# fwereade/trivy

Measured on AMD Instinct MI355X. Metric: packages matched/sec (node), higher is better.
Workload: dtype u8; 1 GPU; c2-dpkg-10000x400; packages=4000000, packages_rank0=4000000, matches_rank0=20482442, kernel_variant=fused_k4_m2400_wseg_rec_r16, db_keys=150005, db_advisories=1709707

## Files before the change

### include/trivy_amd.h

```cpp
#ifndef TRIVY_AMD_H
#define TRIVY_AMD_H

#include <stddef.h>
#include <stdint.h>

#ifdef __cplusplus
extern "C" {
#endif

#define TVM_ABI_VERSION 1

enum {
  TVM_OK = 0,
  TVM_EDETECT = 1,
  TVM_EUNSUPPORTED_OS = 2,
  TVM_EINVAL = 3,
  TVM_EDEVICE = 4,
  TVM_EUNSUPPORTED_TYPE = 5,
};

typedef struct tvm_db tvm_db;
typedef struct tvm_engine tvm_engine;
typedef struct tvm_batch tvm_batch;

// ... 95 lines not shown
int tvm_ospkg_is_supported(const char* os_family, const char* os_ver, int64_t now_unix);
void tvm_result_free(tvm_result* r);

const char* tvm_library_type(const char* lib_type);
int tvm_library_detect(tvm_engine* e, const char* lib_type, const tvm_package* pkgs, size_t n, tvm_result* out,
                       char* err, size_t errlen);
int tvm_library_detect_vulnerabilities(tvm_engine* e, const char* lib_type, tvm_str pkg_id, tvm_str pkg_name,
                                       tvm_str pkg_ver, tvm_result* out, char* err, size_t errlen);

tvm_batch* tvm_batch_new(void);
void tvm_batch_free(tvm_batch* b);
int64_t tvm_batch_add(tvm_batch* b, tvm_engine* e, const char* bucket, tvm_str name, tvm_str version);
enum { TVM_ATTR_ARCH = 1, TVM_ATTR_KSPLICE = 2, TVM_ATTR_CPESET = 4 };
int64_t tvm_batch_add_many_ex(tvm_batch* b, tvm_engine* e, const char* bucket, size_t n, const char* arena,
                              const uint64_t* name_off, const uint32_t* name_len, const uint64_t* ver_off,
                              const uint32_t* ver_len, const uint64_t* arch_off, const uint32_t* arch_len,
                              uint32_t flags);
int64_t tvm_batch_cpe_set(tvm_batch* b, tvm_engine* e, const tvm_str* content_sets, size_t n, tvm_str nvr);
typedef struct {
  const uint64_t* arch_off;
  const uint32_t* arch_len;
  const uint32_t* cpe_set;
} tvm_attr_cols;
int64_t tvm_batch_add_many_attrs(tvm_batch* b, tvm_engine* e, const char* bucket, size_t n, const char* arena,
                                 const uint64_t* name_off, const uint32_t* name_len, const uint64_t* ver_off,
                                 const uint32_t* ver_len, const tvm_attr_cols* attrs, uint32_t flags);
int64_t tvm_batch_add_many(tvm_batch* b, tvm_engine* e, const char* bucket, size_t n, const char* arena,
                           const uint64_t* name_off, const uint32_t* name_len, const uint64_t* ver_off,
                           const uint32_t* ver_len);
int64_t tvm_batch_add_targets(tvm_batch* b, tvm_engine* e, size_t n_targets, const tvm_str* buckets,
                              const uint64_t* target_end, const char* arena, const uint64_t* name_off,
                              const uint32_t* name_len, const uint64_t* ver_off, const uint32_t* ver_len);
int64_t tvm_batch_add_targets_attrs(tvm_batch* b, tvm_engine* e, size_t n_targets, const tvm_str* buckets,
                                    const uint32_t* target_flags, const uint64_t* target_end, const char* arena,
                                    const uint64_t* name_off, const uint32_t* name_len, const uint64_t* ver_off,
                                    const uint32_t* ver_len, const tvm_attr_cols* attrs);
int64_t tvm_batch_size(const tvm_batch* b);
int tvm_batch_upload(tvm_engine* e, tvm_batch* b, uint64_t match_cap, char* err, size_t errlen);
int tvm_match_launch(tvm_engine* e, tvm_batch* b, char* err, size_t errlen);
int tvm_engine_sync(tvm_engine* e, char* err, size_t errlen);
int tvm_device_sync(int device, char* err, size_t errlen);
void tvm_shutdown(void);
int tvm_match_status(tvm_engine* e, tvm_batch* b, uint64_t* n_matches, int64_t* err_pkg, uint64_t* err_bits);
int tvm_match_fetch(tvm_engine* e, tvm_batch* b, uint32_t* pairs, uint64_t cap, uint64_t* n_out);
int tvm_match_copy_device(tvm_engine* e, tvm_batch* b, void* dst, uint64_t cap, uint64_t* n_out);
int tvm_match_order_into(tvm_engine* e, tvm_batch* b, void* csr_adv_dev, void* row_end_dev, uint64_t cap,
                         uint64_t* n_out, char* err, size_t errlen);
int tvm_match_time(tvm_engine* e, tvm_batch* b, int steps, double* ms, char* err, size_t errlen);
uint64_t tvm_match_algorithmic_bytes(tvm_engine* e, tvm_batch* b);
int tvm_version_key(int grammar, const char* s, size_t n, uint8_t* out, size_t cap);
int tvm_version_class(int grammar, const char* s, size_t n);
int tvm_deb_fast_key_host(const char* s, size_t n, uint32_t shift, uint8_t* out, size_t cap);
int tvm_deb_fast_key_slot_host(const char* s, size_t n, uint32_t shift, uint8_t* kb, size_t kb_len);
enum { TVM_ISVULN_PAIRWISE = 0x100 };
int tvm_lib_is_vulnerable_host(int grammar, const char* ver, size_t ver_len, const char* advisory_json,
                               size_t json_len);
const char* tvm_db_advisory_vuln_id(const tvm_db* db, uint32_t adv);

int tvm_db_rows_many(const tvm_db* db, const char* bucket, size_t n, const char* arena, const uint64_t* name_off,
                     const uint32_t* name_len, uint32_t* out);
int tvm_batch_set_package_base(tvm_batch* b, uint32_t base);
int tvm_batch_upload_into(tvm_engine* e, tvm_batch* b, void* pkg_dev, void* adv_dev, uint64_t cap, char* err,
                          size_t errlen);

enum { TVM_PIPE_RAW = 1, TVM_PIPE_ADV32 = 2, TVM_PIPE_RH_MERGE = 4 };
int tvm_pipeline_prepare(tvm_engine* e, tvm_batch* b, uint64_t match_cap, uint32_t chunk_packages, uint32_t flags,
                         char* err, size_t errlen);
int tvm_pipeline_run(tvm_engine* e, tvm_batch* b, uint64_t* n_matches, int64_t* err_pkg, double* ms, char* err,
                     size_t errlen);
int tvm_pipeline_result(tvm_batch* b, const uint32_t** adv, const uint32_t** row_end, uint64_t* n_matches);
int tvm_pipeline_result_raw(tvm_batch* b, const void** adv, uint32_t* width, const uint32_t** row_end,
                            uint64_t* n_matches);
int tvm_pipeline_stats(tvm_batch* b, uint64_t out[5]);
int tvm_wire_encode(size_t n, const uint32_t* plat, const char* arena, const uint64_t* name_off, const uint32_t* name_len,
                    const uint64_t* ver_off, const uint32_t* ver_len, uint32_t chunk_packages, int threads, void* out,
                    uint64_t cap, uint64_t* bytes,
                    uint64_t* chunks, uint64_t chunks_cap, uint64_t* n_chunks, uint32_t* plats, uint32_t plats_cap,
                    uint32_t* n_plats);
int tvm_pipeline_times(tvm_batch* b, uint64_t* encode_us, uint64_t* prepare_us);
void tvm_pool_stats(uint64_t out[4]);
void tvm_pool_trim(void);
int tvm_runtime_info(int* hip_runtime, int* hip_driver, char* path, size_t pathlen);

typedef struct tvm_sbom tvm_sbom;
enum { TVM_SBOM_BORROW = 1 };
int tvm_sbom_decode_cyclonedx(const char* text, size_t len, uint32_t flags, tvm_sbom** out, char* err, size_t errlen);
void tvm_sbom_free(tvm_sbom* s);
int tvm_sbom_info(const tvm_sbom* s, int32_t* has_os, tvm_str* os_family, tvm_str* os_name, tvm_str* serial,
                  int64_t* version, size_t* n_apps);
int tvm_sbom_packages(const tvm_sbom* s, int64_t app, tvm_str* type, tvm_str* file_path, const tvm_package** pkgs,
                      size_t* n);
typedef struct {
  tvm_str purl, bom_ref, layer_digest, layer_diff_id;
  uint32_t present;
} tvm_sbom_extra;
int tvm_sbom_package_extra(const tvm_sbom* s, int64_t app, size_t i, tvm_sbom_extra* out);

int tvm_match_redhat_result(tvm_engine* e, tvm_batch* b, tvm_result* out, char* err, size_t errlen);
int tvm_match_redhat_merge(tvm_engine* e, tvm_batch* b, char* err, size_t errlen);
int tvm_match_redhat_vulns(tvm_engine* e, tvm_batch* b, const uint32_t* pairs, uint64_t n, tvm_result* out,
                           char* err, size_t errlen);
int tvm_match_redhat_merge_time(tvm_engine* e, tvm_batch* b, int steps, double* ms, char* err, size_t errlen);

typedef struct {
  const uint32_t* row_end;
  size_t n_pkgs;
// ... 94 lines not shown
```

### trivy_amd/_lib.py

```python
import atexit
import ctypes
import os

_HERE = os.path.dirname(os.path.abspath(__file__))
LIB_PATH = os.environ.get("TVM_LIB_PATH") or os.path.join(_HERE, "libtrivy_amd.so")

TVM_OK, TVM_EDETECT, TVM_EUNSUPPORTED_OS, TVM_EINVAL, TVM_EDEVICE, TVM_EUNSUPPORTED_TYPE = 0, 1, 2, 3, 4, 5
COPY_PKG_ID, COPY_PKG_NAME, COPY_IDENTIFIER, COPY_LAYER = 1, 2, 4, 8


class Str(ctypes.Structure):
    _fields_ = [("p", ctypes.c_char_p), ("n", ctypes.c_size_t)]


class Package(ctypes.Structure):
    _fields_ = [
        ("id", Str), ("name", Str), ("version", Str), ("release", Str), ("arch", Str),
        ("epoch", ctypes.c_int64),
        ("src_name", Str), ("src_version", Str), ("src_release", Str),
        ("src_epoch", ctypes.c_int64),
        ("modularitylabel", Str),
        ("has_build_info", ctypes.c_int32),
        ("content_sets", ctypes.POINTER(Str)), ("n_content_sets", ctypes.c_size_t),
        ("nvr", Str), ("build_arch", Str),
# ... 152 lines not shown
    ("tvm_engine_sync", ctypes.c_int, [_P, ctypes.c_char_p, ctypes.c_size_t]),
    ("tvm_device_sync", ctypes.c_int, [ctypes.c_int, ctypes.c_char_p, ctypes.c_size_t]),
    ("tvm_shutdown", None, []),
    ("tvm_pipeline_times", ctypes.c_int, [_P, ctypes.POINTER(ctypes.c_uint64), ctypes.POINTER(ctypes.c_uint64)]),
    ("tvm_pool_stats", None, [ctypes.POINTER(ctypes.c_uint64)]),
    ("tvm_sbom_decode_cyclonedx", ctypes.c_int, [ctypes.c_void_p, ctypes.c_size_t, ctypes.c_uint32,
                                                 ctypes.POINTER(ctypes.c_void_p),
                                                 ctypes.c_char_p, ctypes.c_size_t]),
    ("tvm_sbom_free", None, [ctypes.c_void_p]),
    ("tvm_sbom_info", ctypes.c_int, [ctypes.c_void_p, ctypes.POINTER(ctypes.c_int32), ctypes.POINTER(RawStr),
                                     ctypes.POINTER(RawStr), ctypes.POINTER(RawStr), ctypes.POINTER(ctypes.c_int64),
                                     ctypes.POINTER(ctypes.c_size_t)]),
    ("tvm_sbom_packages", ctypes.c_int, [ctypes.c_void_p, ctypes.c_int64, ctypes.POINTER(RawStr), ctypes.POINTER(RawStr),
                                         ctypes.POINTER(ctypes.POINTER(RawPackage)), ctypes.POINTER(ctypes.c_size_t)]),
    ("tvm_sbom_package_extra", ctypes.c_int, [ctypes.c_void_p, ctypes.c_int64, ctypes.c_size_t,
                                              ctypes.POINTER(SbomExtra)]),
    ("tvm_wire_encode", ctypes.c_int, [ctypes.c_size_t, ctypes.c_void_p, ctypes.c_char_p, ctypes.c_void_p,
                                       ctypes.c_void_p, ctypes.c_void_p, ctypes.c_void_p,
                                       ctypes.c_uint32, ctypes.c_int, ctypes.c_void_p, ctypes.c_uint64,
                                       ctypes.POINTER(ctypes.c_uint64), ctypes.c_void_p, ctypes.c_uint64,
                                       ctypes.POINTER(ctypes.c_uint64), ctypes.c_void_p, ctypes.c_uint32,
                                       ctypes.POINTER(ctypes.c_uint32)]),
    ("tvm_pool_trim", None, []),
    ("tvm_match_status", ctypes.c_int, [_P, _P, ctypes.POINTER(ctypes.c_uint64), ctypes.POINTER(ctypes.c_int64),
                                        ctypes.POINTER(ctypes.c_uint64)]),
    ("tvm_match_fetch", ctypes.c_int, [_P, _P, ctypes.c_void_p, ctypes.c_uint64, ctypes.POINTER(ctypes.c_uint64)]),
    ("tvm_match_copy_device", ctypes.c_int, [_P, _P, ctypes.c_void_p, ctypes.c_uint64, ctypes.POINTER(ctypes.c_uint64)]),
    ("tvm_match_order_into", ctypes.c_int, [_P, _P, ctypes.c_void_p, ctypes.c_void_p, ctypes.c_uint64,
                                            ctypes.POINTER(ctypes.c_uint64), ctypes.c_char_p, ctypes.c_size_t]),
    ("tvm_match_time", ctypes.c_int, [_P, _P, ctypes.c_int, ctypes.POINTER(ctypes.c_double), ctypes.c_char_p,
                                      ctypes.c_size_t]),
    ("tvm_match_algorithmic_bytes", ctypes.c_uint64, [_P, _P]),
    ("tvm_db_rows_many", ctypes.c_int, [_P, ctypes.c_char_p, ctypes.c_size_t, ctypes.c_void_p, ctypes.c_void_p,
                                        ctypes.c_void_p, ctypes.c_void_p]),
    ("tvm_batch_set_package_base", ctypes.c_int, [_P, ctypes.c_uint32]),
    ("tvm_batch_upload_into", ctypes.c_int, [_P, _P, ctypes.c_void_p, ctypes.c_void_p, ctypes.c_uint64,
                                             ctypes.c_char_p, ctypes.c_size_t]),
    ("tvm_pipeline_prepare", ctypes.c_int, [_P, _P, ctypes.c_uint64, ctypes.c_uint32, ctypes.c_uint32, ctypes.c_char_p,
                                            ctypes.c_size_t]),
    ("tvm_pipeline_run", ctypes.c_int, [_P, _P, ctypes.POINTER(ctypes.c_uint64), ctypes.POINTER(ctypes.c_int64),
                                        ctypes.POINTER(ctypes.c_double), ctypes.c_char_p, ctypes.c_size_t]),
    ("tvm_pipeline_result", ctypes.c_int, [_P, ctypes.POINTER(ctypes.c_void_p), ctypes.POINTER(ctypes.c_void_p),
                                           ctypes.POINTER(ctypes.c_uint64)]),
    ("tvm_pipeline_result_raw", ctypes.c_int, [_P, ctypes.POINTER(ctypes.c_void_p), ctypes.POINTER(ctypes.c_uint32),
                                               ctypes.POINTER(ctypes.c_void_p), ctypes.POINTER(ctypes.c_uint64)]),
    ("tvm_pipeline_stats", ctypes.c_int, [_P, ctypes.POINTER(ctypes.c_uint64)]),
    ("tvm_version_key", ctypes.c_int, [ctypes.c_int, ctypes.c_char_p, ctypes.c_size_t, ctypes.c_void_p,
                                       ctypes.c_size_t]),
    ("tvm_engine_dropin_stats", ctypes.c_int, [_P, ctypes.POINTER(ctypes.c_uint64)]),
    ("tvm_deb_fast_key_host", ctypes.c_int, [ctypes.c_char_p, ctypes.c_size_t, ctypes.c_uint32, ctypes.c_void_p,
                                             ctypes.c_size_t]),
    ("tvm_deb_fast_key_slot_host", ctypes.c_int, [ctypes.c_char_p, ctypes.c_size_t, ctypes.c_uint32, ctypes.c_void_p,
                                                  ctypes.c_size_t]),
    ("tvm_db_advisory_vuln_id", ctypes.c_char_p, [_P, ctypes.c_uint32]),
    ("tvm_version_class", ctypes.c_int, [ctypes.c_int, ctypes.c_char_p, ctypes.c_size_t]),
    ("tvm_lib_is_vulnerable_host", ctypes.c_int, [ctypes.c_int, ctypes.c_char_p, ctypes.c_size_t, ctypes.c_char_p,
                                                  ctypes.c_size_t]),
    ("tvm_library_type", ctypes.c_char_p, [ctypes.c_char_p]),
    ("tvm_library_detect", ctypes.c_int, [_P, ctypes.c_char_p, ctypes.POINTER(Package), ctypes.c_size_t,
                                          ctypes.POINTER(Result), ctypes.c_char_p, ctypes.c_size_t]),
    ("tvm_library_detect_vulnerabilities", ctypes.c_int, [_P, ctypes.c_char_p, Str, Str, Str, ctypes.POINTER(Result),
                                                          ctypes.c_char_p, ctypes.c_size_t]),
    ("tvm_fill_info", ctypes.c_int, [_P, ctypes.POINTER(FillIn), ctypes.c_size_t, ctypes.POINTER(FillResult),
                                     ctypes.c_char_p, ctypes.c_size_t]),
    ("tvm_fill_result_free", None, [ctypes.POINTER(FillResult)]),
    ("tvm_match_fill", ctypes.c_int, [_P, _P, ctypes.c_char_p, ctypes.c_size_t]),
    ("tvm_match_fill_fetch", ctypes.c_int, [_P, _P, ctypes.c_void_p, ctypes.c_uint64, ctypes.POINTER(ctypes.c_uint64)]),
    ("tvm_match_fill_time", ctypes.c_int, [_P, _P, ctypes.c_int, ctypes.POINTER(ctypes.c_double), ctypes.c_char_p,
                                           ctypes.c_size_t]),
    ("tvm_match_fill_algorithmic_bytes", ctypes.c_uint64, [_P, _P]),
    ("tvm_fill_source_name", ctypes.c_char_p, [_P, ctypes.c_uint32]),
    ("tvm_match_filter", ctypes.c_int, [_P, _P, ctypes.POINTER(FilterOpts), ctypes.POINTER(ctypes.c_uint64),
                                        ctypes.POINTER(ctypes.c_uint64), ctypes.c_char_p, ctypes.c_size_t]),
    ("tvm_match_filter_fetch", ctypes.c_int, [_P, _P, ctypes.c_void_p, ctypes.c_uint64,
                                              ctypes.POINTER(ctypes.c_uint64)]),
    ("tvm_match_filter_ignored", ctypes.c_int, [_P, _P, ctypes.c_void_p, ctypes.c_uint64,
                                                ctypes.POINTER(ctypes.c_uint64)]),
    ("tvm_vuln_rank_many", ctypes.c_int, [_P, ctypes.POINTER(Str), ctypes.c_size_t, ctypes.c_void_p]),
    ("tvm_batch_set_report", ctypes.c_int, [_P, ctypes.c_uint64, ctypes.c_uint64, ctypes.POINTER(Str),
                                            ctypes.POINTER(Str), ctypes.POINTER(Str)]),
    ("tvm_match_vulns", ctypes.c_int, [_P, _P, ctypes.POINTER(VulnSet), ctypes.c_char_p, ctypes.c_size_t]),
    ("tvm_runtime_info", ctypes.c_int, [ctypes.c_void_p, ctypes.c_void_p, ctypes.c_char_p, ctypes.c_size_t]),
    ("tvm_vuln_set_walk", ctypes.c_int, [ctypes.POINTER(VulnSet), _P, ctypes.c_void_p, ctypes.c_void_p]),
    ("tvm_pipeline_vulns", ctypes.c_int, [_P, _P, ctypes.POINTER(VulnSet), ctypes.c_char_p, ctypes.c_size_t]),
    ("tvm_vuln_set_free", None, [ctypes.POINTER(VulnSet)]),
    ("tvm_batch_report_get", ctypes.c_int, [_P, ctypes.c_uint64, ctypes.c_uint64, ctypes.POINTER(RawStr),
                                            ctypes.POINTER(RawStr), ctypes.POINTER(RawStr)]),
    ("tvm_match_filter_time", ctypes.c_int, [_P, _P, ctypes.POINTER(FilterOpts), ctypes.c_int,
                                             ctypes.POINTER(ctypes.c_double), ctypes.c_char_p, ctypes.c_size_t]),
    ("tvm_pipeline_set_filter", ctypes.c_int, [_P, _P, ctypes.POINTER(FilterOpts), ctypes.c_char_p, ctypes.c_size_t]),
    ("tvm_pipeline_filter_stats", ctypes.c_int, [_P, ctypes.POINTER(ctypes.c_uint64)]),
]

EXPORTED = [s[0] for s in _SIG]

_lib = None


def lib():
    global _lib
    if _lib is None:
        if not os.path.exists(LIB_PATH):
            raise RuntimeError(f"trivy_amd native library not built: {LIB_PATH} (run __graft_entry__.build())")
        L = ctypes.CDLL(LIB_PATH)
        for name, res, args in _SIG:
            f = getattr(L, name)
# ... 27 lines not shown
```

### trivy_amd/csrc/capi.cpp

```cpp
#include "../../include/trivy_amd.h"

#include <dlfcn.h>

#include <algorithm>
#include <atomic>
#include <chrono>
#include <cstdio>
#include <cstring>
#include <deque>
#include <memory>
#include <mutex>
#include <new>
#include <shared_mutex>
#include <string>
#include <unordered_map>
#include <vector>

#include "db.h"
#include "drivers.h"
#include "export.h"
#include "engine.h"
#include "libdb.h"
#include "libver.h"
#include "bbolt.h"
// ... 1053 lines not shown

int tvm_version_key(int grammar, const char* s, size_t n, uint8_t* out, size_t cap) {
  struct Sink {
    uint8_t* o;
    size_t cap, n = 0;
    void put(uint8_t b) {
      if (n < cap) o[n] = b;
      n++;
    }
  } sink{out, cap};
  if (grammar <= 0 || grammar > 255 || !s) return -1;
  uint32_t cls = 0;
  if (!encode_version_cls(uint8_t(grammar), reinterpret_cast<const uint8_t*>(s), uint32_t(n), sink, cls)) return -1;
  return int(sink.n);
}

int tvm_version_class(int grammar, const char* s, size_t n) {
  struct Sink {
    void put(uint8_t) {}
  } sink;
  uint32_t cls = 0;
  if (grammar <= 0 || grammar > 255 || !s) return -1;
  if (!encode_version_cls(uint8_t(grammar), reinterpret_cast<const uint8_t*>(s), uint32_t(n), sink, cls)) return -1;
  return int(cls);
}

int tvm_deb_fast_key_host(const char* s, size_t n, uint32_t shift, uint8_t* out, size_t cap) {
  if (!s || n > 4096 || shift > 3) return -3;
  uint8_t tab[128];
  for (uint32_t c = 0; c < 128; c++) tab[c] = deb_fast_code(c);
  std::vector<uint32_t> buf((shift + n) / 4 + 4, 0xA5A5A5A5u);
  uint8_t* b = reinterpret_cast<uint8_t*>(buf.data()) + shift;
  std::memcpy(b, s, n);
  uint8_t kb[kFastKeyStride];
  std::memset(kb, 0xEE, sizeof kb);
  uint32_t len = 0;
  const uint32_t st = deb_fast_key(b, uint32_t(n), kb, tab, len);
  if (st == FAST_INVALID) return -1;
  if (st == FAST_FALLBACK) return -2;
  for (uint32_t i = 0; i < len && i < cap; i++) out[i] = kb[i];
  return int(len);
}

int tvm_deb_fast_key_slot_host(const char* s, size_t n, uint32_t shift, uint8_t* kb, size_t kb_len) {
  if (!s || !kb || n > 4096 || shift > 3 || kb_len < kFastKeyStride) return -3;
  uint8_t tab[128];
  for (uint32_t c = 0; c < 128; c++) tab[c] = deb_fast_code(c);
  std::vector<uint32_t> buf((shift + n) / 4 + 4, 0xA5A5A5A5u);
  uint8_t* b = reinterpret_cast<uint8_t*>(buf.data()) + shift;
  std::memcpy(b, s, n);
  uint32_t len = 0;
  const uint32_t st = deb_fast_key(b, uint32_t(n), kb, tab, len);
  return st == FAST_INVALID ? -1 : st == FAST_FALLBACK ? -2 : int(len);
}

int tvm_lib_is_vulnerable_host(int grammar, const char* ver, size_t ver_len, const char* advisory_json,
                               size_t json_len) {
  Advisory a;
  std::string e;
  if (!ver || !advisory_json || !decode_advisory(std::string_view(advisory_json, json_len), a, e)) return -1;
  const bool pairwise = (grammar & TVM_ISVULN_PAIRWISE) != 0;
  grammar &= ~TVM_ISVULN_PAIRWISE;
  if (grammar == CMP_MAVEN && (pairwise || !mvn_hybrid(a.vulnerable, a.patched, a.unaffected)))
    return mvn_is_vulnerable(a.vulnerable, a.patched, a.unaffected, std::string(ver, ver_len));
  const LibRows r = lib_compile_advisory(uint8_t(grammar), a.vulnerable, a.patched, a.unaffected);
  return lib_rows_contain(uint8_t(grammar), r, std::string(ver, ver_len)) ? 1 : 0;
}

int tvm_library_detect(tvm_engine* e, const char* lib_type, const tvm_package* pkgs, size_t n, tvm_result* out,
                       char* err, size_t errlen) {
  if (!e || !lib_type || !out || (n && !pkgs)) return TVM_EINVAL;
  memset(out, 0, sizeof(*out));
  std::shared_lock<std::shared_mutex> lk(e->mu);
  std::vector<Pkg> p = to_pkgs(pkgs, n);
  std::vector<Vuln> vulns;
  std::string msg;
  const DetectStatus st = library_detect(*e->eng, lib_type, p, vulns, msg);
  if (st == DETECT_UNSUPPORTED_OS) return TVM_EUNSUPPORTED_TYPE;
  if (st != DETECT_OK) {
    set_err(err, errlen, msg);
    return TVM_EDETECT;
  }
  export_result(e->eng->db(), std::move(vulns), false, out);
  return TVM_OK;
}

int tvm_library_detect_vulnerabilities(tvm_engine* e, const char* lib_type, tvm_str pkg_id, tvm_str pkg_name,
                                       tvm_str pkg_ver, tvm_result* out, char* err, size_t errlen) {
  if (!e || !lib_type || !out) return TVM_EINVAL;
  memset(out, 0, sizeof(*out));
  std::shared_lock<std::shared_mutex> lk(e->mu);
  std::vector<Pkg> p(1);
  p[0].id = sv(pkg_id);
  p[0].name = sv(pkg_name);
  p[0].version = sv(pkg_ver);
  std::vector<Vuln> vulns;
  std::string msg;
  const DetectStatus st = library_detect_vulnerabilities(*e->eng, lib_type, p, vulns, msg);
  if (st == DETECT_UNSUPPORTED_OS) return TVM_EUNSUPPORTED_TYPE;
  if (st != DETECT_OK) {
    set_err(err, errlen, msg);
    return TVM_EDETECT;
  }
  export_result(e->eng->db(), std::move(vulns), false, out);
  return TVM_OK;
}
// ... 1335 lines not shown
```

### trivy_amd/csrc/match_kernel.h

```cpp
#pragma once
#include "engine.h"
#include "libver.h"
#include "match_variants.h"

namespace tvm {

constexpr uint32_t kStage = 12288;
constexpr uint32_t kKeyWords = 4;
constexpr uint32_t kMapCap = 4096;

struct ProbeArgs {
  DevDB db;
  const uint2* pk;
  const uint64_t* tile_off;
  const uint8_t* arena;
  uint32_t n;
  uint32_t p0;
  uint32_t n_total;
  PkgRec* rec;
  uint4* tail;
  unsigned long long* ctl;
  uint64_t* spill;
  uint64_t spill_cap;
};
// ... 108 lines not shown
  const uintptr_t a = reinterpret_cast<uintptr_t>(s);
  const P* base = reinterpret_cast<const P*>(a & ~uintptr_t(3));
  const uint32_t sh = uint32_t(a & 3);
  uint64_t h = key_hash_seed2(plat, n);
  for (uint32_t i = 0; 8 * i < n; i++) h = key_hash_word(h, name_word(base, sh, i, n));
  return key_hash_fin(h);
}

template <class P>
__device__ __forceinline__ bool name_eq_slot(const uint8_t* s, uint32_t n, const uint4 q1, const uint4 q2,
                                             const uint4 q3, const uint8_t* arena) {
  static_assert(kSlotNameWords == 4, "four inline name words (q3.z / q3.w: Slot::pfx)");
  const uintptr_t a = reinterpret_cast<uintptr_t>(s);
  const P* base = reinterpret_cast<const P*>(a & ~uintptr_t(3));
  const uint32_t sh = uint32_t(a & 3);
  const uint64_t y[kSlotNameWords] = {q1.z | (uint64_t(q1.w) << 32), q2.x | (uint64_t(q2.y) << 32),
                                      q2.z | (uint64_t(q2.w) << 32), q3.x | (uint64_t(q3.y) << 32)};
  bool eq = true;
#pragma unroll
  for (uint32_t i = 0; i < kSlotNameWords; i++) eq &= (8 * i < n ? name_word(base, sh, i, n) : 0ull) == y[i];
  if (eq && n > 8 * kSlotNameWords) {
    const uint8_t* full = arena + q1.y;
    for (uint32_t i = 8 * kSlotNameWords; eq && i < n; i++) eq = full[i] == s[i];
  }
  return eq;
}

template <class P>
__device__ __forceinline__ void probe_lookup(const ProbeArgs& a, uint32_t p, uint32_t plat, const PlatInfo& pi,
                                            uint32_t nlen, const uint8_t* name, bool valid, uint64_t h,
                                            uint64_t start, bool found, uint4 q0, uint4 q0n, bool has_q0n,
                                            uint32_t& rbeg, uint32_t& cnt, uint32_t* sflags = nullptr,
                                            uint32_t cls = 0, uint64_t* pfx = nullptr);

__device__ __forceinline__ uint4 slot_head(const ProbeArgs& a, uint64_t i) {
  return reinterpret_cast<const uint4*>(a.db.slots + (i & a.db.slot_mask))[0];
}

__device__ __forceinline__ bool fp_chain(const ProbeArgs& a, uint64_t h, uint64_t& i) {
  i = h & a.db.slot_mask;
#ifdef TVM_EXP_NOFP
  return true;
#else
  const uint8_t want = slot_fp_of(h);
  for (;;) {
    const uint8_t f = a.db.slot_fp[i];
    if (f == 0) return false;
    if (f == want) return true;
    i = (i + 1) & a.db.slot_mask;
  }
#endif
}

template <uint32_t GM, class P, int DIAG = 0>
__device__ __forceinline__ void probe_one(const ProbeArgs& a, uint32_t p, uint32_t plat, uint32_t nlen, uint32_t vlen,
                                          const uint8_t* name, const uint8_t* ver, uint64_t vglob, PkgRec& r,
                                          uint8_t* kb = nullptr, const uint8_t* tab = nullptr) {
  const PlatInfo pi = a.db.plats[plat];
  constexpr bool kPre = GM == GM_DEB;
  uint64_t h = 0, start = 0;
  bool found = false;
  uint4 q0 = make_uint4(0, 0, 0, 0), q0n = q0;
  bool has_q0n = false;
  if (!(DIAG & 2)) {
    h = name_hash<P>(plat, name, nlen);
    found = fp_chain(a, h, start);
  }
  auto heads = [&]() {
    if ((DIAG & 2) || !found) return;
    q0 = slot_head(a, start);
    if constexpr (kPre) {
      has_q0n = !(start & 1);
      if (has_q0n) q0n = slot_head(a, start + 1);
    }
  };
  if constexpr (kPre) heads();
  if (!(DIAG & 1) && kb && ((GM >> CMP_DEB) & 1u) && pi.cmp == CMP_DEB) {
    uint32_t kl = 0;
    const uint32_t st = deb_fast_key(ver, vlen, kb, tab, kl);
    if (st != FAST_FALLBACK) {
      const bool valid = st == FAST_OK;
      const uint32_t* kw = reinterpret_cast<const uint32_t*>(kb);
      uint32_t kinfo = (valid ? (kl & KI_LEN) | KI_VALID : 0u) | KI_H24, koff = 0;
      r.k0 = r.k1 = r.k2 = 0;
      if (valid) {
        const uint64_t m0 = uint64_t(kw[0]) | (uint64_t(kw[1]) << 32), m1 = uint64_t(kw[2]) | (uint64_t(kw[3]) << 32);
        r.k0 = be_word(m0, kl < 8 ? kl : 8);
        r.k1 = kl > 8 ? be_word(m1, kl < 16 ? kl - 8 : 8) : 0ull;
        r.k2 = kl > 16 ? be_word(uint64_t(kw[4]) | (uint64_t(kw[5]) << 32), kl < 24 ? kl - 16 : 8) : 0ull;
        static_assert(kFastKeyCap <= kKeyWords * 8, "fast keys fit head + tail slot");
        if (kl > (GM == GM_DEB ? 24u : 16u)) a.tail[p] = make_uint4(kw[4], kw[5], kw[6], kw[7]);
      }
      uint32_t cnt = 0, rbeg = 0;
      if constexpr (!kPre) heads();
      uint64_t pfx = 0;
      if (!(DIAG & 2)) probe_lookup<P>(a, p, plat, pi, nlen, name, (kinfo & KI_VALID) != 0, h, start, found, q0, q0n, has_q0n,
                                          rbeg, cnt, nullptr, 0, GM == GM_DEB ? &pfx : nullptr);
      if constexpr (GM == GM_DEB)
        kinfo |= ((uint32_t(pfx) & KI_P_MASK) << KI_P_SHIFT) | (row16_prefix_cmp(r.k0, kl, pfx) << KI_PFX_SHIFT);
      r.meta = make_uint4(rbeg, cnt, kinfo, koff);
      return;
    }
  }
  uint64_t* tslot = reinterpret_cast<uint64_t*>(a.tail + p);
  HeadSink hs(tslot);
  uint32_t cls = 0;
  bool valid = true;
  if (DIAG & 1) {
    hs.n = vlen;
    hs.w0 = vlen;
  } else {
    valid = encode_version_gm<GM>(pi.cmp, ver, vlen, hs, cls);
  }
  hs.flush();
  uint32_t kinfo = 0, koff = 0;
  const bool mvn_pkg = ((GM >> CMP_MAVEN) & 1u) && pi.cmp == CMP_MAVEN;
  if (valid && hs.n > (mvn_pkg ? 16u : kKeyWords * 8)) {
    const uint32_t need = (hs.n + 7) / 8;
    const unsigned long long o = atomicAdd(&a.ctl[2], (unsigned long long)need);
    if (o + need > a.spill_cap) {
      atomicOr(&a.ctl[3], (unsigned long long)ERR_SPILL);
      valid = false;
    } else {
      WordSink ws(a.spill + o);
      uint32_t cls2 = 0;
      encode_version_gm<GM>(pi.cmp, ver, vlen, ws, cls2);
      ws.flush();
      koff = uint32_t(o);
      kinfo |= KI_SPILL;
    }
  }
  uint32_t cnt = 0, rbeg = 0, sflags = 0;
// ... 636 lines not shown
  const bool mvn = FILT >= 2 && dq.cap && __syncthreads_or((r.meta.z & KI_MVN) != 0);
  const uint32_t nm = sweep<K, MB, FILT, false>(a, s, madv, mq, map, nnz, total, tid, 0, mvn, dq);

  if (tid == 0) {
    s.base = nm ? atomicAdd(&a.ctl[0], (unsigned long long)nm) : 0ull;
    TileDir e;
    e.base = s.base;
    e.count = nm;
    e.pad = 0;
    a.dir[a.t0 + t] = e;
  }
  __syncthreads();
  const unsigned long long base = s.base;
  if (nm <= uint32_t(MB)) {
    const uint32_t pb = a.out_base + a.p0 + t * kTile;
    for (uint32_t i = tid; i < nm; i += kTile) {
      if (base + i < a.out_cap) {
        a.out_pkg[base + i] = pb + mq[i];
        a.out_adv[base + i] = madv[i];
      }
    }
  } else {
    sweep<K, MB, FILT, true>(a, s, madv, mq, map, nnz, total, tid, base, mvn, dq);
  }
}

template <int K, int MB, int FILT>
__global__ __launch_bounds__(kTile) void sweep_kernel(SweepArgs a) {
  __shared__ SweepShared<FILT> s;
  __shared__ uint32_t madv[MB];
  __shared__ uint8_t mq[MB];
  __shared__ uint8_t map[kMapCap];
  constexpr uint32_t kQ = FILT >= 2 ? 512 : 1;
  __shared__ uint32_t dqj[kQ], dqres[FILT >= 2 ? kTile / 8 : 1];
  const uint32_t tid = threadIdx.x, t = blockIdx.x;
  const uint32_t p = t * kTile + tid;
  PkgRec r;
  r.meta = make_uint4(0, 0, 0, 0);
  r.k0 = r.k1 = r.k2 = 0;
  if (p < a.n) r = a.rec[p];
  sweep_tile<K, MB, FILT>(a, s, madv, mq, map, t, tid, r, DeferQ{dqj, dqres, FILT >= 2 ? kQ : 0u});
}

template <uint32_t GM, int K, int MB, int FILT, int DIAG = 0, int WPE = 1, int SEG = 0, uint32_t STG = kStage,
          bool MOVE = false>
__global__ __launch_bounds__(kTile, WPE) void fused_kernel(FusedArgs fa) {
  constexpr uint32_t kStageVec = STG / 16 + 8;
  constexpr uint32_t kMbufVec = (MB * 5 + 15) / 16;
  __shared__ uint4 buf[kStageVec > kMbufVec ? kStageVec : kMbufVec];
  struct SweepPart {
    SweepShared<FILT> s;
    uint8_t map[kMapCap];
  };
  struct ProbePart {
    uint32_t kbuf[kTile * kFastKeyStride / 4];
    uint8_t tab[128];
  };
  static_assert(sizeof(ProbePart) <= sizeof(SweepPart), "the probe's LDS fits in the sweep's");
  __shared__ union {
    SweepPart sw;
    ProbePart pr;
  } u;
  SweepShared<FILT>& s = u.sw.s;
  uint8_t* map = u.sw.map;
  constexpr bool kHot = ((SEG >> 2) & 3) == 3;
  __shared__ uint64_t hot_head[kHot ? kTile : 1];
  __shared__ uint32_t hot_tail[kHot ? kTile : 1];
  const ProbeArgs& a = fa.pa;
  if constexpr (MOVE) {
    if (blockIdx.x < fa.n_copy) {
      static_assert(sizeof(buf) >= kCopyLdsWords * 4, "the result move borrows the staging buffer");
      __builtin_amdgcn_s_setprio(3);
      copy_out_tiles(fa.co, blockIdx.x, fa.n_copy, reinterpret_cast<uint32_t*>(buf));
      return;
    }
  }
  const uint32_t tid = threadIdx.x;
  if (!MOVE && fa.ctl_zero && blockIdx.x == 0 && tid < 8) fa.ctl_zero[tid] = 0ull;
  const uint32_t t = MOVE ? blockIdx.x - fa.n_copy : (fa.tile_map ? fa.tile_map[blockIdx.x] : blockIdx.x);
  const uint32_t p = t * kTile + tid;
  uint2 d = make_uint2(0xFFFFFFFFu, 0);
  if (p < a.n) d = a.pk[p];
  constexpr bool kWaveStage = (SEG & 2) != 0;
  const uint32_t g = t * kGroupsPerTile + (kWaveStage ? (tid >> 6) : 0u);
  const uint64_t w0 = a.tile_off[g], w1 = a.tile_off[kWaveStage ? g + 1 : (t + 1) * kGroupsPerTile];
  const uint32_t nlen = d.y & 0xFFFFu, vlen = d.y >> 16;
  uint32_t off = 0;
  uint4* sbuf = buf;
  const uint64_t base16 = w0 & ~uint64_t(15);
  bool staged;
  if constexpr (kWaveStage) {
    off = wave_exscan(nlen + vlen, tid & 63);
    sbuf = buf + (tid >> 6) * (STG / 4 / 16 + 2);
    staged = w1 - base16 <= STG / 4;
    if (staged) stage_window_wave<STG>(sbuf, a.arena + base16, uint32_t((w1 - base16 + 15) / 16), tid & 63);
    if (tid < 128) u.pr.tab[tid] = deb_fast_code(tid);
    __syncthreads();
  } else {
    block_exscan<kTile>(s.wsum[0], nlen + vlen, tid, off);
    staged = w1 - base16 <= STG;
    if (staged) stage_window<STG>(buf, a.arena + base16, uint32_t((w1 - base16 + 15) / 16), tid);
    if (tid < 128) u.pr.tab[tid] = deb_fast_code(tid);
    __syncthreads();
  }
  PkgRec r;
  r.meta = make_uint4(0, 0, 0, 0);
  r.k0 = r.k1 = r.k2 = 0;
  if (p < a.n && d.x < a.db.n_plats) {
    if (staged) {
      const uint8_t* sb = reinterpret_cast<const uint8_t*>(sbuf) + uint32_t(w0 - base16) + off;
      probe_one<GM, uint32_t, DIAG & 3>(a, p, d.x, nlen, vlen, sb, sb + nlen, w0 + off + nlen, r,
                                        reinterpret_cast<uint8_t*>(u.pr.kbuf) + tid * kFastKeyStride, u.pr.tab);
    } else {
      const uint8_t* gb = a.arena + w0 + off;
      probe_one<GM, uint32_t, DIAG & 3>(a, p, d.x, nlen, vlen, gb, gb + nlen, w0 + off + nlen, r);
    }
  }
  if (DIAG & 4) r.meta.y = 0;
  __syncthreads();
  uint32_t* madv = reinterpret_cast<uint32_t*>(buf);
  constexpr uint32_t kBufWords = sizeof(buf) / 4, kMbWords = (uint32_t(MB) * 5 + 3) / 4;
  constexpr uint32_t kQ = kBufWords > kMbWords + kTile / 8 + 16 ? kBufWords - kMbWords - kTile / 8 : 0;
  static_assert(FILT < 2 || kQ >= 16, "no room for the Maven program queue");
  const DeferQ dq{madv + kMbWords + kTile / 8, madv + kMbWords, FILT >= 2 ? kQ : 0u};
  sweep_tile<K, MB, FILT, SEG>(fa.sa, s, madv, reinterpret_cast<uint8_t*>(madv + MB), map, t, tid, r, dq,
                               Hot16{hot_head, hot_tail});
}

template <uint32_t GM, int DIAG = 0>
void launch_probe(uint32_t n_tiles, hipStream_t st, const ProbeArgs& a) {
  hipLaunchKernelGGL((probe_kernel<GM, DIAG>), dim3(n_tiles), dim3(kTile), 0, st, a);
}

template <int K, int MB, int FILT>
void launch_sweep(uint32_t n_tiles, hipStream_t st, const SweepArgs& a) {
  hipLaunchKernelGGL((sweep_kernel<K, MB, FILT>), dim3(n_tiles), dim3(kTile), 0, st, a);
}

template <uint32_t GM, int K, int MB, int FILT, int DIAG = 0, int WPE = 1, int SEG = 0, uint32_t STG = kStage>
void launch_fused(uint32_t n_tiles, hipStream_t st, const FusedArgs& a) {
  if (a.n_copy)
    hipLaunchKernelGGL((fused_kernel<GM, K, MB, FILT, DIAG, WPE, SEG, STG, true>), dim3(n_tiles + a.n_copy), dim3(kTile), 0,
                       st, a);
  else
    hipLaunchKernelGGL((fused_kernel<GM, K, MB, FILT, DIAG, WPE, SEG, STG, false>), dim3(n_tiles), dim3(kTile), 0, st, a);
}

template <uint32_t GM, int FILT, int F, int K, int MB>
constexpr FusedFn fused_entry() {
  if constexpr (F == 0) return nullptr;
  else if constexpr (F == 4) return &launch_fused<GM, K, MB, FILT, 0, 1, 1>;
  else if constexpr (F == 5) return &launch_fused<GM, K, MB, FILT, 0, 1, 3>;
  else if constexpr (F == 6) return &launch_fused<GM, K, MB, FILT, 0, 6, 3>;
  else if constexpr (F == 7) {
    if constexpr (GM == GM_DEB) return &launch_fused<GM, K, MB, FILT, 0, 1, 3 | 12>;
    else return nullptr;
  } else if constexpr (F == 8) {
    if constexpr (GM == GM_DEB) return &launch_fused<GM, K, MB, FILT, 0, 1, 3 | 12 | 16>;
    else return nullptr;
  } else if constexpr (F == 25 || F == 26) {
    if constexpr (GM == GM_DEB) return &launch_fused<GM, K, MB, FILT, 0, 1, 3 | (F == 25 ? 4 : 8)>;
    else return nullptr;
  }
  else return &launch_fused<GM, K, MB, FILT, (F >= 10 ? F - 10 : 0), (FILT >= 2 && K <= 2 && F == 1) ? 5 : TVM_FUSED_WPE(F)>;
}

}
}
```

### trivy_amd/csrc/match_variants.h

```cpp
#pragma once

#define TVM_MATCH_VARIANTS_PRODUCT(X)  \
  X(1, 4, 2048, "fused_k4_m2048")      \
  X(1, 2, 2048, "fused_k2_m2048")      \
  X(1, 1, 2048, "fused_k1_m2048")      \
  X(0, 2, 2048, "split_k2_m2048")      \
  X(0, 4, 2048, "split_k4_m2048")      \
  X(4, 4, 2400, "fused_k4_m2400_seg")  \
  X(5, 4, 2400, "fused_k4_m2400_wseg")  \
  X(6, 2, 2400, "fused_k2_m2400_wseg6") \
  X(6, 3, 2400, "fused_k3_m2400_wseg6") \
  X(7, 4, 2400, "fused_k4_m2400_wseg_r16") \
  X(7, 8, 2400, "fused_k8_m2400_wseg_r16") \
  X(8, 4, 2400, "fused_k4_m2400_wseg_rec_r16")

#ifdef TVM_DIAG
#define TVM_MATCH_VARIANTS(X)      \
  TVM_MATCH_VARIANTS_PRODUCT(X)    \
  X(11, 4, 2048, "diag_no_encode") \
  X(12, 4, 2048, "diag_no_probe")  \
  X(14, 4, 2048, "diag_no_sweep")  \
  X(15, 4, 2048, "diag_stage_only") \
  X(25, 4, 2400, "diag_row16_k4")  \
  X(25, 8, 2400, "diag_row16_k8")  \
  X(26, 4, 2400, "diag_row16s_k4")
#else
#define TVM_MATCH_VARIANTS(X) TVM_MATCH_VARIANTS_PRODUCT(X)
#endif

#define TVM_FUSED_WPE(F) ((F) == 2 ? 6 : (F) == 3 ? 8 : 1)

#define TVM_VARIANT_COUNT_(F, K, MB, NAME) +1
constexpr int kNumTuned = 0 TVM_MATCH_VARIANTS(TVM_VARIANT_COUNT_);
#undef TVM_VARIANT_COUNT_

constexpr int kAutoVariant = 11;
constexpr int kAutoVariantFiltered = 1;
constexpr int kAutoVariantOS = 7;
constexpr int kAutoVariantLean = 7;
```

### trivy_amd/csrc/verkey.h

```cpp
#pragma once
#include "common.h"
#include "unicode_tab.h"

namespace tvm {

static __constant__ uint32_t d_uni_letter[TVM_UNI_NLETTER][2] = {TVM_UNI_LETTER_RANGES};
static __constant__ uint32_t d_uni_digit[TVM_UNI_NDIGIT][2] = {TVM_UNI_DIGIT_RANGES};
static const uint32_t h_uni_letter[TVM_UNI_NLETTER][2] = {TVM_UNI_LETTER_RANGES};
static const uint32_t h_uni_digit[TVM_UNI_NDIGIT][2] = {TVM_UNI_DIGIT_RANGES};

TVM_HD bool uni_in(const uint32_t (*t)[2], int n, uint32_t cp) {
  int lo = 0, hi = n - 1;
  while (lo <= hi) {
    int mid = (lo + hi) >> 1;
    if (cp < t[mid][0]) hi = mid - 1;
    else if (cp > t[mid][1]) lo = mid + 1;
    else return true;
  }
  return false;
}
TVM_HD bool rune_letter(uint32_t cp) {
  if (cp < 0x80) return ((cp | 0x20) >= 'a' && (cp | 0x20) <= 'z');
#ifdef __HIP_DEVICE_COMPILE__
  return uni_in(d_uni_letter, TVM_UNI_NLETTER, cp);
// ... 283 lines not shown
      if (d >= 10) return FAST_FALLBACK;
      epoch = epoch * 10u + d;
    }
    r0 = colon + 1;
  }
  const bool has_rev = dash < n && dash >= r0;
  if (r0 >= (has_rev ? dash : n) || uint32_t(s[r0]) - '0' >= 10u) return FAST_INVALID;
  if (has_rev && lcolon < n && lcolon > dash) return FAST_INVALID;
  const uint32_t ke = epoch ? (39u - uint32_t(__builtin_clz(epoch))) >> 3 : 0u;
  const uint32_t eb = ke ? epoch << (32 - 8 * ke) : 0u;
  kb[0] = uint8_t(ke);
  kb[1] = uint8_t(eb >> 24);
  kb[2] = uint8_t(eb >> 16);
  kb[3] = uint8_t(eb >> 8);
  kb[4] = uint8_t(eb);
  uint32_t pos = 1 + ke;
  DebFastState st{pos, 0u, false, false, false};
  const uint8_t* s2 = s + r0;
  const uint32_t m = n - r0, sp2 = has_rev ? dash - r0 : 0xFFFFFFFFu;
  const uintptr_t a2 = reinterpret_cast<uintptr_t>(s2);
  const uint32_t* base2 = reinterpret_cast<const uint32_t*>(a2 & ~uintptr_t(3));
  const uint32_t sh2 = uint32_t(a2 & 3);
  for (uint32_t j = 0; j + 4 <= m; j += 4) {
    const uint32_t x = str_dword(base2, sh2, j >> 2);
#pragma unroll
    for (uint32_t b = 0; b < 4; b++) deb_fast_byte((x >> (8 * b)) & 0xFFu, j + b == sp2, kb, tab, st);
  }
  for (uint32_t j = m & ~3u; j < m; j++) deb_fast_byte(s2[j], j == sp2, kb, tab, st);
  if (st.bad) return FAST_INVALID;
  if (st.ovf) return FAST_FALLBACK;
  pos = st.pos;
  const uint32_t v = st.v;
  {
    const uint32_t k = (39u - clz32(v)) >> 3;
    const uint32_t vb = v << ((32u - 8u * k) & 31u);
    uint8_t* o = kb + (pos < kFastKeyCap ? pos : kFastKeyCap);
    o[0] = uint8_t(DEB_TERM0 + k);
    o[1] = uint8_t(vb >> 24);
    o[2] = uint8_t(vb >> 16);
    o[3] = uint8_t(vb >> 8);
    o[4] = uint8_t(vb);
    pos += k + 1;
    kb[pos < kFastKeyCap ? pos : kFastKeyCap] = DEB_END;
    pos++;
    if (!has_rev) {
      kb[pos < kFastKeyCap ? pos : kFastKeyCap] = DEB_TERM0;
      kb[pos + 1 < kFastKeyCap ? pos + 1 : kFastKeyCap] = DEB_END;
      pos += 2;
    }
  }
  if (pos > kFastKeyCap) return FAST_FALLBACK;
  len = pos;
  return FAST_OK;
}

template <class Sink>
TVM_HD void put_sint(int64_t v, Sink& o) {
  if (v >= 0) {
    const uint64_t u = uint64_t(v);
    uint32_t k = 0;
    for (uint64_t t = u; t; t >>= 8) k++;
    o.put(uint8_t(0x80 + k));
    for (int b = int(k) - 1; b >= 0; b--) o.put(uint8_t(u >> (8 * b)));
  } else {
    const uint64_t m = ~uint64_t(v);
    uint32_t k = 0;
    for (uint64_t t = m; t; t >>= 8) k++;
    o.put(uint8_t(0x7F - k));
    for (int b = int(k) - 1; b >= 0; b--) o.put(uint8_t(~(m >> (8 * b))));
  }
}

enum : int { APK_INVALID = -1, APK_DOZ = 0, APK_DIGIT, APK_LETTER, APK_SUFFIX, APK_SUFFIX_NO, APK_REV, APK_END };
enum : uint8_t {
  APKC_SUFPRE = 0x01, APKC_END = 0x02, APKC_REV = 0x03, APKC_SUFNO = 0x04, APKC_SUFPOST = 0x05,
  APKC_LETTER = 0x06, APKC_DIGIT = 0x07, APKC_DOZ = 0x08,
};

TVM_HD bool apk_lower(uint8_t c) { return c >= 'a' && c <= 'z'; }

TVM_HD int apk_next_kind(int kind, const uint8_t* s, uint32_t n, uint32_t& i) {
  int k = APK_INVALID;
  if (i >= n || s[i] == 0) {
    k = APK_END;
  } else if ((kind == APK_DIGIT || kind == APK_DOZ) && apk_lower(s[i])) {
    k = APK_LETTER;
  } else if (kind == APK_LETTER && is_adigit(s[i])) {
    k = APK_DIGIT;
  } else if (kind == APK_SUFFIX && is_adigit(s[i])) {
    k = APK_SUFFIX_NO;
  } else {
    if (s[i] == '.') k = APK_DOZ;
    else if (s[i] == '_') k = APK_SUFFIX;
    else if (s[i] == '-') {
      if (i + 1 < n && s[i + 1] == 'r') {
        k = APK_REV;
        i++;
      }
    }
    i++;
  }
  if (k < kind && !((k == APK_DOZ && kind == APK_DIGIT) || (k == APK_SUFFIX && kind == APK_SUFFIX_NO) ||
                    (k == APK_DIGIT && kind == APK_LETTER)))
    k = APK_INVALID;
  return k;
}
// ... 222 lines not shown
```

Before: 10.91 billion packages/s.

## Balance dpkg version-key encoding across lanes by sorting work into length buckets

Adds a balanced fused-kernel variant for dpkg that first computes name hashes and chain heads per lane, then buckets the packages needing fast-key encoding by version length in LDS. Threads are reassigned so that lanes of a wave encode similar-length versions together, which cuts divergence in the deb_fast_key loop. The encoded status and length go into spare slot bytes and are read back by the owning lane, which then probes using the precomputed state. The cost is extra LDS, atomics, and additional __syncthreads. The auto-selected variant index now points at the new variant.

```diff
diff --git a/include/trivy_amd.h b/include/trivy_amd.h
--- a/include/trivy_amd.h
+++ b/include/trivy_amd.h
@@ -171,6 +171,9 @@
 int tvm_version_class(int grammar, const char* s, size_t n);
 int tvm_deb_fast_key_host(const char* s, size_t n, uint32_t shift, uint8_t* out, size_t cap);
 int tvm_deb_fast_key_slot_host(const char* s, size_t n, uint32_t shift, uint8_t* kb, size_t kb_len);
+int tvm_enc_bal_buckets_host(void);
+int tvm_enc_bal_bucket_host(uint32_t version_len);
+int tvm_enc_bal_item_host(const uint32_t* counts, uint32_t item, uint32_t* bucket, uint32_t* index);
 enum { TVM_ISVULN_PAIRWISE = 0x100 };
 int tvm_lib_is_vulnerable_host(int grammar, const char* ver, size_t ver_len, const char* advisory_json,
                                size_t json_len);
diff --git a/trivy_amd/_lib.py b/trivy_amd/_lib.py
--- a/trivy_amd/_lib.py
+++ b/trivy_amd/_lib.py
@@ -228,6 +228,10 @@
                                              ctypes.c_size_t]),
     ("tvm_deb_fast_key_slot_host", ctypes.c_int, [ctypes.c_char_p, ctypes.c_size_t, ctypes.c_uint32, ctypes.c_void_p,
                                                   ctypes.c_size_t]),
+    ("tvm_enc_bal_buckets_host", ctypes.c_int, []),
+    ("tvm_enc_bal_bucket_host", ctypes.c_int, [ctypes.c_uint32]),
+    ("tvm_enc_bal_item_host", ctypes.c_int, [ctypes.POINTER(ctypes.c_uint32), ctypes.c_uint32,
+                                             ctypes.POINTER(ctypes.c_uint32), ctypes.POINTER(ctypes.c_uint32)]),
     ("tvm_db_advisory_vuln_id", ctypes.c_char_p, [_P, ctypes.c_uint32]),
     ("tvm_version_class", ctypes.c_int, [ctypes.c_int, ctypes.c_char_p, ctypes.c_size_t]),
     ("tvm_lib_is_vulnerable_host", ctypes.c_int, [ctypes.c_int, ctypes.c_char_p, ctypes.c_size_t, ctypes.c_char_p,
diff --git a/trivy_amd/csrc/capi.cpp b/trivy_amd/csrc/capi.cpp
--- a/trivy_amd/csrc/capi.cpp
+++ b/trivy_amd/csrc/capi.cpp
@@ -1129,6 +1129,17 @@
   uint32_t len = 0;
   const uint32_t st = deb_fast_key(b, uint32_t(n), kb, tab, len);
   return st == FAST_INVALID ? -1 : st == FAST_FALLBACK ? -2 : int(len);
+}
+
+int tvm_enc_bal_buckets_host(void) { return int(kEncBuckets); }
+int tvm_enc_bal_bucket_host(uint32_t version_len) { return int(enc_bal_bucket(version_len)); }
+int tvm_enc_bal_item_host(const uint32_t* counts, uint32_t item, uint32_t* bucket, uint32_t* index) {
+  if (!counts || !bucket || !index) return -1;
+  uint32_t b = 0, i = 0;
+  if (!enc_bal_item(counts, item, b, i)) return 0;
+  *bucket = b;
+  *index = i;
+  return 1;
 }
 
 int tvm_lib_is_vulnerable_host(int grammar, const char* ver, size_t ver_len, const char* advisory_json,
diff --git a/trivy_amd/csrc/match_kernel.h b/trivy_amd/csrc/match_kernel.h
--- a/trivy_amd/csrc/match_kernel.h
+++ b/trivy_amd/csrc/match_kernel.h
@@ -184,17 +184,33 @@
 #endif
 }
 
-template <uint32_t GM, class P, int DIAG = 0>
+struct ProbePre {
+  uint64_t h, start;
+  uint4 q0, q0n;
+  bool found, has_q0n;
+  uint32_t fast_st, fast_kl;
+};
+
+template <uint32_t GM, class P, int DIAG = 0, int PRE = 0>
 __device__ __forceinline__ void probe_one(const ProbeArgs& a, uint32_t p, uint32_t plat, uint32_t nlen, uint32_t vlen,
                                           const uint8_t* name, const uint8_t* ver, uint64_t vglob, PkgRec& r,
-                                          uint8_t* kb = nullptr, const uint8_t* tab = nullptr) {
+                                          uint8_t* kb = nullptr, const uint8_t* tab = nullptr,
+                                          const ProbePre* pre = nullptr) {
   const PlatInfo pi = a.db.plats[plat];
   constexpr bool kPre = GM == GM_DEB;
   uint64_t h = 0, start = 0;
   bool found = false;
   uint4 q0 = make_uint4(0, 0, 0, 0), q0n = q0;
   bool has_q0n = false;
-  if (!(DIAG & 2)) {
+  if constexpr (PRE != 0) {
+    static_assert(GM == GM_DEB && DIAG == 0, "the balanced kernel is dpkg-only");
+    h = pre->h;
+    start = pre->start;
+    found = pre->found;
+    q0 = pre->q0;
+    q0n = pre->q0n;
+    has_q0n = pre->has_q0n;
+  } else if (!(DIAG & 2)) {
     h = name_hash<P>(plat, name, nlen);
     found = fp_chain(a, h, start);
   }
@@ -206,10 +222,15 @@
       if (has_q0n) q0n = slot_head(a, start + 1);
     }
   };
-  if constexpr (kPre) heads();
+  if constexpr (kPre && PRE == 0) heads();
   if (!(DIAG & 1) && kb && ((GM >> CMP_DEB) & 1u) && pi.cmp == CMP_DEB) {
-    uint32_t kl = 0;
-    const uint32_t st = deb_fast_key(ver, vlen, kb, tab, kl);
+    uint32_t kl = 0, st;
+    if constexpr (PRE == 2) {
+      st = pre->fast_st;
+      kl = pre->fast_kl;
+    } else {
+      st = deb_fast_key(ver, (DIAG & 8) ? min(vlen, 12u) : vlen, kb, tab, kl);
+    }
     if (st != FAST_FALLBACK) {
       const bool valid = st == FAST_OK;
       const uint32_t* kw = reinterpret_cast<const uint32_t*>(kb);
@@ -952,9 +973,15 @@
     SweepShared<FILT> s;
     uint8_t map[kMapCap];
   };
+  constexpr bool kBal = (SEG & 32) != 0;
+  static_assert(!kBal || (GM == GM_DEB && (SEG & 2) && DIAG == 0), "encoder balance: dpkg-only, per-wave staging");
   struct ProbePart {
     uint32_t kbuf[kTile * kFastKeyStride / 4];
     uint8_t tab[128];
+    uint32_t bal_cnt[kBal ? kEncBuckets : 1];
+    uint32_t bal_mixed;
+    uint32_t bal_ver[kBal ? kTile : 1];
+    uint8_t bal_list[kBal ? kEncBuckets * kTile : 1];
   };
   static_assert(sizeof(ProbePart) <= sizeof(SweepPart), "the probe's LDS fits in the sweep's");
   __shared__ union {
@@ -984,17 +1011,51 @@
   constexpr bool kWaveStage = (SEG & 2) != 0;
   const uint32_t g = t * kGroupsPerTile + (kWaveStage ? (tid >> 6) : 0u);
   const uint64_t w0 = a.tile_off[g], w1 = a.tile_off[kWaveStage ? g + 1 : (t + 1) * kGroupsPerTile];
+  if constexpr (kBal) {
+    if (tid < kEncBuckets) u.pr.bal_cnt[tid] = 0;
+    if (tid == kEncBuckets) u.pr.bal_mixed = 0;
+    __syncthreads();
+  }
   const uint32_t nlen = d.y & 0xFFFFu, vlen = d.y >> 16;
   uint32_t off = 0;
   uint4* sbuf = buf;
   const uint64_t base16 = w0 & ~uint64_t(15);
   bool staged;
+  const bool own = p < a.n && d.x < a.db.n_plats;
+  ProbePre pre;
+  pre.h = pre.start = 0;
+  pre.q0 = pre.q0n = make_uint4(0, 0, 0, 0);
+  pre.found = pre.has_q0n = false;
+  pre.fast_st = pre.fast_kl = 0;
+  bool listed = false;
   if constexpr (kWaveStage) {
     off = wave_exscan(nlen + vlen, tid & 63);
     sbuf = buf + (tid >> 6) * (STG / 4 / 16 + 2);
     staged = w1 - base16 <= STG / 4;
     if (staged) stage_window_wave<STG>(sbuf, a.arena + base16, uint32_t((w1 - base16 + 15) / 16), tid & 63);
     if (tid < 128) u.pr.tab[tid] = deb_fast_code(tid);
+    if constexpr (kBal) {
+      if (!staged) {
+        if ((tid & 63) == 0) u.pr.bal_mixed = 1;
+      } else if (own) {
+        const uint32_t noff = uint32_t(reinterpret_cast<const uint8_t*>(sbuf) - reinterpret_cast<const uint8_t*>(buf)) +
+                              uint32_t(w0 - base16) + off;
+        pre.h = name_hash<uint32_t>(d.x, reinterpret_cast<const uint8_t*>(buf) + noff, nlen);
+        pre.found = fp_chain(a, pre.h, pre.start);
+        if (pre.found) {
+          pre.q0 = slot_head(a, pre.start);
+          pre.has_q0n = !(pre.start & 1);
+          if (pre.has_q0n) pre.q0n = slot_head(a, pre.start + 1);
+          listed = a.db.plats[d.x].cmp == CMP_DEB;
+          if (listed) {
+            const uint32_t b = enc_bal_bucket(vlen);
+            const uint32_t rank = atomicAdd(&u.pr.bal_cnt[b], 1u);
+            u.pr.bal_list[b * kTile + rank] = uint8_t(tid);
+            u.pr.bal_ver[tid] = (noff + nlen) | (vlen << 16);
+          }
+        }
+      }
+    }
     __syncthreads();
   } else {
     block_exscan<kTile>(s.wsum[0], nlen + vlen, tid, off);
@@ -1006,11 +1067,45 @@
   PkgRec r;
   r.meta = make_uint4(0, 0, 0, 0);
   r.k0 = r.k1 = r.k2 = 0;
-  if (p < a.n && d.x < a.db.n_plats) {
+  if constexpr (kBal) {
+    uint8_t* const kbytes = reinterpret_cast<uint8_t*>(u.pr.kbuf);
+    const uint8_t* sb = reinterpret_cast<const uint8_t*>(sbuf) + uint32_t(w0 - base16) + off;
+    const bool packed = u.pr.bal_mixed == 0;
+    if (packed) {
+      uint32_t cnt[kEncBuckets];
+#pragma unroll
+      for (uint32_t i = 0; i < kEncBuckets; i++) cnt[i] = u.pr.bal_cnt[i];
+      uint32_t b = 0, idx = 0;
+      if (enc_bal_item(cnt, tid, b, idx)) {
+        const uint32_t q = u.pr.bal_list[b * kTile + idx], e = u.pr.bal_ver[q];
+        uint8_t* kb = kbytes + q * kFastKeyStride;
+        uint32_t kl = 0;
+        const uint32_t st = deb_fast_key(reinterpret_cast<const uint8_t*>(buf) + (e & 0xFFFFu), e >> 16, kb, u.pr.tab, kl);
+        static_assert(kFastKeyStride == 44 && kFastKeyCap + 5 <= 40, "slot bytes 40..43 are free");
+        reinterpret_cast<uint32_t*>(kb)[10] = st | (kl << 8);
+      }
+      __syncthreads();
+    }
+    if (packed && listed) {
+      const uint32_t w = reinterpret_cast<const uint32_t*>(kbytes + tid * kFastKeyStride)[10];
+      pre.fast_st = w & 0xFFu;
+      pre.fast_kl = w >> 8;
+      probe_one<GM, uint32_t, 0, 2>(a, p, d.x, nlen, vlen, sb, sb + nlen, w0 + off + nlen, r,
+                                    kbytes + tid * kFastKeyStride, u.pr.tab, &pre);
+    } else if (own && (!packed || pre.found)) {
+      if (staged) {
+        probe_one<GM, uint32_t, 0>(a, p, d.x, nlen, vlen, sb, sb + nlen, w0 + off + nlen, r,
+                                   kbytes + tid * kFastKeyStride, u.pr.tab);
+      } else {
+        const uint8_t* gb = a.arena + w0 + off;
+        probe_one<GM, uint32_t, 0>(a, p, d.x, nlen, vlen, gb, gb + nlen, w0 + off + nlen, r);
+      }
+    }
+  } else if (p < a.n && d.x < a.db.n_plats) {
     if (staged) {
       const uint8_t* sb = reinterpret_cast<const uint8_t*>(sbuf) + uint32_t(w0 - base16) + off;
-      probe_one<GM, uint32_t, DIAG & 3>(a, p, d.x, nlen, vlen, sb, sb + nlen, w0 + off + nlen, r,
-                                        reinterpret_cast<uint8_t*>(u.pr.kbuf) + tid * kFastKeyStride, u.pr.tab);
+      probe_one<GM, uint32_t, DIAG & 11>(a, p, d.x, nlen, vlen, sb, sb + nlen, w0 + off + nlen, r,
+                                         reinterpret_cast<uint8_t*>(u.pr.kbuf) + tid * kFastKeyStride, u.pr.tab);
     } else {
       const uint8_t* gb = a.arena + w0 + off;
       probe_one<GM, uint32_t, DIAG & 3>(a, p, d.x, nlen, vlen, gb, gb + nlen, w0 + off + nlen, r);
@@ -1058,9 +1153,15 @@
   } else if constexpr (F == 8) {
     if constexpr (GM == GM_DEB) return &launch_fused<GM, K, MB, FILT, 0, 1, 3 | 12 | 16>;
     else return nullptr;
+  } else if constexpr (F == 9) {
+    if constexpr (GM == GM_DEB) return &launch_fused<GM, K, MB, FILT, 0, 1, 3 | 12 | 16 | 32>;
+    else return nullptr;
   } else if constexpr (F == 25 || F == 26) {
     if constexpr (GM == GM_DEB) return &launch_fused<GM, K, MB, FILT, 0, 1, 3 | (F == 25 ? 4 : 8)>;
     else return nullptr;
+  } else if constexpr (F == 28) {
+    if constexpr (GM == GM_DEB) return &launch_fused<GM, K, MB, FILT, 8, 1, 3 | 12 | 16>;
+    else return nullptr;
   }
   else return &launch_fused<GM, K, MB, FILT, (F >= 10 ? F - 10 : 0), (FILT >= 2 && K <= 2 && F == 1) ? 5 : TVM_FUSED_WPE(F)>;
 }
diff --git a/trivy_amd/csrc/match_variants.h b/trivy_amd/csrc/match_variants.h
--- a/trivy_amd/csrc/match_variants.h
+++ b/trivy_amd/csrc/match_variants.h
@@ -12,7 +12,8 @@
   X(6, 3, 2400, "fused_k3_m2400_wseg6") \
   X(7, 4, 2400, "fused_k4_m2400_wseg_r16") \
   X(7, 8, 2400, "fused_k8_m2400_wseg_r16") \
-  X(8, 4, 2400, "fused_k4_m2400_wseg_rec_r16")
+  X(8, 4, 2400, "fused_k4_m2400_wseg_rec_lane_r16") \
+  X(9, 4, 2400, "fused_k4_m2400_wseg_rec_r16")
 
 #ifdef TVM_DIAG
 #define TVM_MATCH_VARIANTS(X)      \
@@ -23,7 +24,8 @@
   X(15, 4, 2048, "diag_stage_only") \
   X(25, 4, 2400, "diag_row16_k4")  \
   X(25, 8, 2400, "diag_row16_k8")  \
-  X(26, 4, 2400, "diag_row16s_k4")
+  X(26, 4, 2400, "diag_row16s_k4") \
+  X(28, 4, 2400, "diag_enc12")
 #else
 #define TVM_MATCH_VARIANTS(X) TVM_MATCH_VARIANTS_PRODUCT(X)
 #endif
@@ -34,7 +36,7 @@
 constexpr int kNumTuned = 0 TVM_MATCH_VARIANTS(TVM_VARIANT_COUNT_);
 #undef TVM_VARIANT_COUNT_
 
-constexpr int kAutoVariant = 11;
+constexpr int kAutoVariant = 12;
 constexpr int kAutoVariantFiltered = 1;
 constexpr int kAutoVariantOS = 7;
 constexpr int kAutoVariantLean = 7;
diff --git a/trivy_amd/csrc/verkey.h b/trivy_amd/csrc/verkey.h
--- a/trivy_amd/csrc/verkey.h
+++ b/trivy_amd/csrc/verkey.h
@@ -359,6 +359,26 @@
   if (pos > kFastKeyCap) return FAST_FALLBACK;
   len = pos;
   return FAST_OK;
+}
+
+constexpr uint32_t kEncBuckets = 8;
+TVM_HD uint32_t enc_bal_bucket(uint32_t n) {
+  const uint32_t d = (n + 3) >> 2;
+  return d < kEncBuckets - 1 ? d : kEncBuckets - 1;
+}
+TVM_HD bool enc_bal_item(const uint32_t* cnt, uint32_t item, uint32_t& bucket, uint32_t& idx) {
+  uint32_t end = 0, first = 0, k = 0;
+#pragma unroll
+  for (uint32_t j = 0; j < kEncBuckets; j++) {
+    end += cnt[kEncBuckets - 1 - j];
+    const bool past = item >= end;
+    first = past ? end : first;
+    k += past ? 1u : 0u;
+  }
+  if (k >= kEncBuckets) return false;
+  bucket = kEncBuckets - 1 - k;
+  idx = item - first;
+  return true;
 }
 
 template <class Sink>
```

Measured after the change: 11.14 billion packages/s (median of 6 runs). 2.2% higher.
